# mauruszach/multimodal_diffusion

Hardware: AMD Instinct MI355X
Metric: denoising steps/sec @256x256 multimodal-cond batch=32 (higher is better)
Workload: dtype f32 via 3xbf16 split operands (6-term products, f32 accumulate; fp32-level error); 1 GPU; C3: 256x256 audio->video CFG denoising step (cond+null MMDiT d512 L8 H8 + noise head + DDIM), 384+37 tokens, batch 32 per GPU, DDIM 50 steps, guidance 3.5; global_batch=32, sampler_steps=50, parallelism=dp1, launch=eager, matmul=bf16x3, attn=default, cfg_halves=one stacked 2B batch, one stream

## Files before the change

multimodal_diffusion_amd/csrc/attn_bf16x3.hip:

```cpp
#include "avd_common.h"

#include <stdlib.h>
#include <type_traits>

namespace avd {

constexpr int A3_DH = 64, A3_KT = 64, A3_NW = 4;
constexpr float A3_NEG = -1.0e30f;

typedef short s16x4 __attribute__((ext_vector_type(4)));
typedef unsigned int u32x2 __attribute__((ext_vector_type(2)));
typedef float f32x4t __attribute__((ext_vector_type(4)));

#define AVD_LDS_PTR(p) ((__attribute__((address_space(3))) void*)(p))
#define AVD_GLB_PTR(p) ((const __attribute__((address_space(1))) void*)(p))

template <int TERMS> struct A3Terms;
template <> struct A3Terms<6> { static constexpr int N = 6; static constexpr int PA[6] = {2, 0, 1, 1, 0, 0}; static constexpr int PB[6] = {0, 2, 1, 0, 1, 0}; };
template <> struct A3Terms<9> { static constexpr int N = 9; static constexpr int PA[9] = {2, 2, 1, 2, 0, 1, 1, 0, 0}; static constexpr int PB[9] = {2, 1, 2, 0, 2, 1, 0, 1, 0}; };
template <> struct A3Terms<1> { static constexpr int N = 1; static constexpr int PA[1] = {0}; static constexpr int PB[1] = {0}; };
template <> struct A3Terms<3> { static constexpr int N = 3; static constexpr int PA[3] = {0, 1, 0}; static constexpr int PB[3] = {1, 0, 0}; };

template <bool SPLIT_OUT, int TERMS>
__global__ __launch_bounds__(A3_NW * 64, 2) void attn_bf16x3_kernel(const unsigned char* __restrict__ img, float* __restrict__ out,
                                                                    int Bt, int N, int Npad, int H, int n_query_max, int nqb,
                                                                    float s_inv2, float v_inv, float o_scale, RowSegs oseg) {
    constexpr int NW = A3_NW, ROWB = QKV3_ROWB;
    constexpr bool F16 = TERMS == 3;
    constexpr int NPL = s3_planes(TERMS);
    constexpr int PPW = 24 / NW;
    __shared__ __attribute__((aligned(16))) unsigned char Ks[A3_KT * ROWB];
    __shared__ __attribute__((aligned(16))) unsigned char Vs[A3_KT * ROWB];

    int qb, h, b;
    {
        const int nwg = gridDim.x, id = blockIdx.x, q = nwg >> 3, r = nwg & 7, x = id & 7;
        const int w = (x < r ? x * (q + 1) : r * (q + 1) + (x - r) * q) + (id >> 3);
        qb = w % nqb;
        h = (w / nqb) % H;
        b = w / (nqb * H);
    }
    const int seg_tok = oseg.tok[b < oseg.samples[0] ? 0 : 1], n_query = n_query_max < seg_tok ? n_query_max : seg_tok;
    if (qb * (A3_NW * 32) >= n_query) return;
    const int tid = threadIdx.x, lane = tid & 63, wave = tid >> 6;
    const int l31 = lane & 31, hi = lane >> 5;
    const int64_t hstride = (int64_t)Npad * ROWB;
    const unsigned char* Qb = img + (((int64_t)0 * Bt + b) * H + h) * hstride;
    const unsigned char* Kb = img + (((int64_t)1 * Bt + b) * H + h) * hstride;
    const unsigned char* Vb = img + (((int64_t)2 * Bt + b) * H + h) * hstride;

    const int q_row = qb * (NW * 32) + wave * 32 + l31;
    bf16x8 qf[4][3];
    {
        const unsigned char* src = Qb + (int64_t)(q_row < N ? q_row : N - 1) * ROWB + hi * 16;
#pragma unroll
        for (int s = 0; s < 4; ++s)
#pragma unroll
            for (int p = 0; p < NPL; ++p) qf[s][p] = *reinterpret_cast<const bf16x8*>(src + p * 128 + s * 32);
    }

    auto dma = [&](const unsigned char* gsrc, unsigned char* ldst, int kt) {
        const int last_row = N - 1 - kt * A3_KT;
#pragma unroll
        for (int i = 0; i < PPW; ++i) {
            const int p = wave + NW * i;
            const int off = p * 1024 + lane * 16;
            int row = off / ROWB;
            const int within = off - row * ROWB;
            row = row < last_row ? row : last_row;
            __builtin_amdgcn_global_load_lds(AVD_GLB_PTR(gsrc + ((int64_t)kt * A3_KT + row) * ROWB + within), AVD_LDS_PTR(ldst + p * 1024), 16,
                                             0, 0);
        }
    };

    f32x16 o0, o1;
#pragma unroll
    for (int r = 0; r < 16; ++r) { o0[r] = 0.f; o1[r] = 0.f; }
    float m_run = A3_NEG, l_run = 0.f;

    const int nkt = (N + A3_KT - 1) / A3_KT;
    dma(Kb, Ks, 0);
    dma(Vb, Vs, 0);
    __builtin_amdgcn_s_waitcnt(0x0f70);
    __syncthreads();

    const int ksw = (l31 >> 1) & 7;
    const int k_rd = l31 * ROWB;
    const int i16 = lane & 15, cb = (lane >> 4) & 1;
    const int v_q = i16 >> 2, v_p = i16 & 3;

    const bool active = qb * (NW * 32) + wave * 32 < n_query;
    for (int kt = 0; kt < nkt; ++kt) {
        const bool more = (kt + 1) < nkt;
        if (!active) {
            __builtin_amdgcn_s_waitcnt(0x0f70);
            __syncthreads();
            if (more) dma(Kb, Ks, kt + 1);
            __builtin_amdgcn_s_waitcnt(0x0f70);
            __syncthreads();
            if (more) dma(Vb, Vs, kt + 1);
            continue;
        }
        f32x16 s0, s1;
#pragma unroll
        for (int r = 0; r < 16; ++r) { s0[r] = 0.f; s1[r] = 0.f; }
        using TT = A3Terms<TERMS>;
#pragma unroll
        for (int s = 0; s < 4; ++s) {
            bf16x8 ka[3], kb2[3];
            const int ch = ((2 * s + hi) ^ ksw) << 4;
#pragma unroll
            for (int p = 0; p < NPL; ++p) {
                ka[p] = *reinterpret_cast<const bf16x8*>(Ks + k_rd + p * 128 + ch);
                kb2[p] = *reinterpret_cast<const bf16x8*>(Ks + k_rd + 32 * ROWB + p * 128 + ch);
            }
#pragma unroll
            for (int t = 0; t < TT::N; ++t) {
                s0 = mma16<F16>(ka[TT::PA[t]], qf[s][TT::PB[t]], s0);
                s1 = mma16<F16>(kb2[TT::PA[t]], qf[s][TT::PB[t]], s1);
            }
        }
        __builtin_amdgcn_s_waitcnt(0x0f70);
        __syncthreads();
        if (more) dma(Kb, Ks, kt + 1);

        if constexpr (F16) {
#pragma unroll
            for (int r = 0; r < 16; ++r) { s0[r] *= s_inv2; s1[r] *= s_inv2; }
        }
        if (!more && (N & (A3_KT - 1))) {
            const int kbase = kt * A3_KT;
#pragma unroll
            for (int r = 0; r < 16; ++r) {
                const int key = kbase + mfma32_row(r, hi);
                if (key >= N) s0[r] = A3_NEG;
                if (key + 32 >= N) s1[r] = A3_NEG;
            }
        }

        float mt = s0[0];
#pragma unroll
        for (int r = 1; r < 16; ++r) mt = fmaxf(mt, s0[r]);
#pragma unroll
        for (int r = 0; r < 16; ++r) mt = fmaxf(mt, s1[r]);
        mt = fmaxf(mt, __shfl_xor(mt, 32, 64));
        const float m_new = fmaxf(m_run, mt);
        const float m_sub = F16 ? m_new - 15.0f : m_new;
        float ps = 0.f;
#pragma unroll
        for (int r = 0; r < 16; ++r) {
            s0[r] = __builtin_amdgcn_exp2f(s0[r] - m_sub);
            s1[r] = __builtin_amdgcn_exp2f(s1[r] - m_sub);
            ps += s0[r] + s1[r];
        }
        if (__any(m_new > m_run)) {
            const float alpha = __builtin_amdgcn_exp2f(m_run - m_new);
// ... 272 lines not shown

    auto tile = [&](auto flags, int kt, f32x16& c0, f32x16& c1, f32x16& n0, f32x16& n1) {
        using FL = decltype(flags);
        constexpr bool MORE = FL::MORE;
        const float m_sub = F16 ? m_new - 15.0f : m_new;
        const float alpha = __builtin_amdgcn_exp2f(m_run - m_new);
        m_run = m_new;
        float ps = 0.f;
        constexpr int NSLOT_A = 4 * TT::N, NITEM_A = 28;
        auto item_a = [&](int w) {
            if (w < 16) {
                const float e0 = F16 ? c0[w] * s_inv2 : c0[w], e1 = F16 ? c1[w] * s_inv2 : c1[w];
                float p0 = __builtin_amdgcn_exp2f(e0 - m_sub), p1 = __builtin_amdgcn_exp2f(e1 - m_sub);
                ps += p0 + p1;
                asm volatile("" : "+v"(p0), "+v"(p1), "+v"(ps));
                c0[w] = p0;
                c1[w] = p1;
            } else if (w < 24) {
                const int r0 = (w - 16) * 2;
                float a0 = o0[r0] * alpha, a1 = o0[r0 + 1] * alpha, q0 = o1[r0] * alpha, q1 = o1[r0 + 1] * alpha;
                asm volatile("" : "+v"(a0), "+v"(a1), "+v"(q0), "+v"(q1));
                o0[r0] = a0; o0[r0 + 1] = a1;
                o1[r0] = q0; o1[r0 + 1] = q1;
            } else {
                split_pair(c0, c1, 0, w - 24, pf[0]);
                if constexpr (NPL == 3) asm volatile("" : "+v"(pf[0][0][w - 24]), "+v"(pf[0][1][w - 24]), "+v"(pf[0][2][w - 24]));
                else if constexpr (NPL == 2) asm volatile("" : "+v"(pf[0][0][w - 24]), "+v"(pf[0][1][w - 24]));
                else asm volatile("" : "+v"(pf[0][0][w - 24]));
            }
        };
        if constexpr (MORE) {
#pragma unroll
            for (int r = 0; r < 16; ++r) { n0[r] = 0.f; n1[r] = 0.f; }
#pragma unroll
            for (int sl = 0; sl < NSLOT_A; ++sl) {
                A3_SB();
                s_slot(n0, n1, sl / TT::N, sl % TT::N);
#pragma unroll
                for (int w = sl * NITEM_A / NSLOT_A; w < (sl + 1) * NITEM_A / NSLOT_A; ++w) item_a(w);
            }
            A3_SB();
            if constexpr (FL::VCL) {
                if (ragged) mask_tail(n0, n1, kt + 1);
            }
        } else {
#pragma unroll
            for (int w = 0; w < NITEM_A; ++w) item_a(w);
        }
        l_run = l_run * alpha + ps;
        sync();
        if constexpr (MORE) {
            if constexpr (FL::KCL) { if (kt + 2 < nkt) dma_clamp(Kb, Ks, kt + 2); }
            else if constexpr (!FL::VCL) dma_full(Kb, Ks, kt + 2);
        }

        float mt = A3_NEG;
#pragma unroll
        for (int g = 0; g < 4; ++g) {
#pragma unroll
            for (int sl = 0; sl < 2 * TT::N; ++sl) {
                A3_SB();
                pv_slot(g, sl / TT::N, sl % TT::N, pf[g & 1]);
                if (g < 3) {
                    constexpr int SPS = 2 * TT::N >= 4 ? 1 : 2;
#pragma unroll
                    for (int e = sl * SPS; e < (sl + 1) * SPS && e < 4; ++e) split_pair(c0, c1, g + 1, e, pf[(g + 1) & 1]);
                }
                if (MORE && g == 3) {
#pragma unroll
                    for (int w = sl * 16 / (2 * TT::N); w < (sl + 1) * 16 / (2 * TT::N); ++w) mt = fmaxf(mt, fmaxf(n0[w], n1[w]));
                    asm volatile("" : "+v"(mt));
                }
            }
        }
        A3_SB();
        if constexpr (MORE) {
            if constexpr (F16) mt *= s_inv2;
            mt = fmaxf(mt, __shfl_xor(mt, 32, 64));
            m_new = fmaxf(m_run, mt);
            if constexpr (FL::COPY) {
                c0 = n0;
                c1 = n1;
            }
            sync();
            if constexpr (FL::VCL) dma_clamp(Vb, Vs, kt + 1);
            else dma_full(Vb, Vs, kt + 1);
        }
    };
    {
        using Main = A3Flags<true, false, false, false>;
        using MainC = A3Flags<true, false, false, true>;
        using KClamp = A3Flags<true, true, false, true>;
        using VClamp = A3Flags<true, false, true, true>;
        using Last = A3Flags<false, false, false, false>;
        int kt = 0;
        for (; kt + 4 < nkt; kt += 2) {
            tile(Main{}, kt, sa0, sa1, sb0, sb1);
            tile(Main{}, kt + 1, sb0, sb1, sa0, sa1);
        }
        if (nkt - kt == 4) { tile(MainC{}, kt, sa0, sa1, sb0, sb1); ++kt; }
        if (nkt - kt == 3) { tile(KClamp{}, kt, sa0, sa1, sb0, sb1); ++kt; }
        if (nkt - kt == 2) { tile(VClamp{}, kt, sa0, sa1, sb0, sb1); ++kt; }
        tile(Last{}, kt, sa0, sa1, sb0, sb1);
    }
#undef A3_SB

    const float l_tot = l_run + __shfl_xor(l_run, 32, 64);
    const float inv = F16 ? v_inv / l_tot : 1.0f / l_tot;
    const int d = H * A3_DH;
    if constexpr (SPLIT_OUT) {
        float ch[8][4];
#pragma unroll
        for (int g4 = 0; g4 < 4; ++g4)
#pragma unroll
            for (int e = 0; e < 4; ++e) {
                ch[g4][e] = o0[4 * g4 + e] * inv;
                ch[4 + g4][e] = o1[4 * g4 + e] * inv;
            }
        unsigned char* o3 = reinterpret_cast<unsigned char*>(out);
#pragma unroll
        for (int c = 0; c < 8; c += 2) {
            float v[8];
#pragma unroll
            for (int e = 0; e < 4; ++e) {
                const float send = hi ? ch[c][e] : ch[c + 1][e];
                const float recv = __shfl_xor(send, 32, 64);
                v[e] = hi ? recv : ch[c][e];
                v[4 + e] = hi ? ch[c + 1][e] : recv;
            }
            if (q_row < n_query) {
                if constexpr (F16) store_split8_h2(o3, oseg.row(b, q_row), h * A3_DH + 8 * (c + hi), d, v, o_scale);
                else store_split8(o3, oseg.row(b, q_row), h * A3_DH + 8 * (c + hi), d, v);
            }
        }
    } else if (q_row < n_query) {
        float* dst = out + (oseg.row(b, q_row)) * d + h * A3_DH + 4 * hi;
#pragma unroll
        for (int g4 = 0; g4 < 4; ++g4) {
            f32x4 a = {o0[4 * g4] * inv, o0[4 * g4 + 1] * inv, o0[4 * g4 + 2] * inv, o0[4 * g4 + 3] * inv};
            f32x4 c = {o1[4 * g4] * inv, o1[4 * g4 + 1] * inv, o1[4 * g4 + 2] * inv, o1[4 * g4 + 3] * inv};
            *reinterpret_cast<f32x4*>(dst + 8 * g4) = a;
            *reinterpret_cast<f32x4*>(dst + 32 + 8 * g4) = c;
        }
    }
}

template <bool F16>
__device__ __forceinline__ f32x4t mma16s(bf16x8 a, bf16x8 b, f32x4t c) {
    if constexpr (F16) return __builtin_amdgcn_mfma_f32_16x16x32_f16(__builtin_bit_cast(f16x8, a), __builtin_bit_cast(f16x8, b), c, 0, 0, 0);
    else return __builtin_amdgcn_mfma_f32_16x16x32_bf16(a, b, c, 0, 0, 0);
}
int g_attn_m16 = 1;

struct S16 { f32x4t t[4][2]; };

template <bool SPLIT_OUT, int TERMS>
__global__ __launch_bounds__(A3_NW * 64, 2) void attn_bf16x3_p16_kernel(const unsigned char* __restrict__ img, float* __restrict__ out,
                                                                        int Bt, int N, int Npad, int H, int n_query_max, int nqb,
                                                                        float s_inv2, float v_inv, float o_scale, RowSegs oseg) {
    constexpr int NW = A3_NW, ROWB = QKV3_ROWB;
    constexpr bool F16 = TERMS == 3;
    constexpr int NPL = s3_planes(TERMS);
    constexpr int PPW = 24 / NW;
    using TT = A3Terms<TERMS>;
    __shared__ __attribute__((aligned(16))) unsigned char Ks[A3_KT * ROWB];
    __shared__ __attribute__((aligned(16))) unsigned char Vs[A3_KT * ROWB];

    int qb, h, b;
    {
        const int nwg = gridDim.x, id = blockIdx.x, q = nwg >> 3, r = nwg & 7, x = id & 7;
        const int w = (x < r ? x * (q + 1) : r * (q + 1) + (x - r) * q) + (id >> 3);
        qb = w % nqb;
        h = (w / nqb) % H;
        b = w / (nqb * H);
    }
    const int seg_tok = oseg.tok[b < oseg.samples[0] ? 0 : 1], n_query = n_query_max < seg_tok ? n_query_max : seg_tok;
    if (qb * (A3_NW * 32) >= n_query) return;
    const int tid = threadIdx.x, lane = tid & 63;
    const int wave = __builtin_amdgcn_readfirstlane(tid >> 6);
    const int l15 = lane & 15, kq = lane >> 4;
    const int64_t hstride = (int64_t)Npad * ROWB;
    const unsigned char* Qb = img + (((int64_t)0 * Bt + b) * H + h) * hstride;
    const unsigned char* Kb = img + (((int64_t)1 * Bt + b) * H + h) * hstride;
    const unsigned char* Vb = img + (((int64_t)2 * Bt + b) * H + h) * hstride;

    const int q_row0 = qb * (NW * 32) + wave * 32 + l15;
    bf16x8 qf[2][2][3];
#pragma unroll
    for (int qt = 0; qt < 2; ++qt) {
        const int qr = q_row0 + 16 * qt;
        const unsigned char* src = Qb + (int64_t)(qr < N ? qr : N - 1) * ROWB + kq * 16;
#pragma unroll
        for (int sd = 0; sd < 2; ++sd)
#pragma unroll
            for (int p = 0; p < NPL; ++p) qf[qt][sd][p] = *reinterpret_cast<const bf16x8*>(src + p * 128 + sd * 64);
    }
    auto dma_clamp = [&](const unsigned char* gsrc, unsigned char* ldst, int kt) {
        const int last_row = N - 1 - kt * A3_KT;
#pragma unroll
        for (int i = 0; i < PPW; ++i) {
            const int p = wave + NW * i;
            const int off = p * 1024 + lane * 16;
            int row = off / ROWB;
            const int within = off - row * ROWB;
            row = row < last_row ? row : last_row;
            __builtin_amdgcn_global_load_lds(AVD_GLB_PTR(gsrc + ((int64_t)kt * A3_KT + row) * ROWB + within), AVD_LDS_PTR(ldst + p * 1024), 16,
                                             0, 0);
        }
    };
    const unsigned lane16 = (unsigned)lane * 16u;
    auto dma_full = [&](const unsigned char* gsrc, unsigned char* ldst, int kt) {
        const unsigned char* base = gsrc + ((int64_t)kt * (A3_KT * ROWB) + wave * 1024);
#pragma unroll
        for (int i = 0; i < PPW; ++i)
            __builtin_amdgcn_global_load_lds(AVD_GLB_PTR(base + i * (NW * 1024) + lane16), AVD_LDS_PTR(ldst + (wave + NW * i) * 1024), 16, 0, 0);
    };
    auto sync = [&]() {
        __builtin_amdgcn_s_waitcnt(0x0f70);
        __syncthreads();
    };

    const int nkt = (N + A3_KT - 1) / A3_KT;
    const bool ragged = (N & (A3_KT - 1)) != 0;
    dma_clamp(Kb, Ks, 0);
    dma_clamp(Vb, Vs, 0);
    sync();

    const bool active = qb * (NW * 32) + wave * 32 < n_query;
    if (!active) {
        sync();
        if (nkt > 1) dma_clamp(Kb, Ks, 1);
        sync();
        for (int kt = 0; kt < nkt; ++kt) {
            sync();
            if (kt + 2 < nkt) dma_clamp(Kb, Ks, kt + 2);
            if (kt + 1 < nkt) {
                sync();
                dma_clamp(Vb, Vs, kt + 1);
            }
        }
        return;
    }

    const int ksw = (l15 >> 1) & 7;
    const int k_rd = l15 * ROWB;
    const int v_q = l15 >> 2, v_p = l15 & 3;
    const int v_key = 4 * kq + v_q;
    const int v_sw = qkv3_swizzle(2, v_key);
    const int v_rd = v_key * ROWB + 8 * (v_p & 1);
#define A3_SB() __builtin_amdgcn_sched_barrier(0)

    f32x4t o[4][2];
    S16 sa, sb;
#pragma unroll
    for (int i = 0; i < 4; ++i)
#pragma unroll
        for (int j = 0; j < 2; ++j) { o[i][j] = f32x4t{0.f, 0.f, 0.f, 0.f}; sa.t[i][j] = o[i][j]; sb.t[i][j] = o[i][j]; }
    float m_run[2] = {A3_NEG, A3_NEG}, l_run[2] = {0.f, 0.f}, m_new[2];

    bf16x8 ka[3];
    auto s_slot = [&](S16& d, int kt4, int sd, int t) {
        if (t == 0) {
            const int ch = ((4 * sd + kq) ^ ksw) << 4;
#pragma unroll
            for (int p = 0; p < NPL; ++p) ka[p] = *reinterpret_cast<const bf16x8*>(Ks + k_rd + kt4 * (16 * ROWB) + p * 128 + ch);
        }
        d.t[kt4][0] = mma16s<F16>(ka[TT::PA[t]], qf[0][sd][TT::PB[t]], d.t[kt4][0]);
        d.t[kt4][1] = mma16s<F16>(ka[TT::PA[t]], qf[1][sd][TT::PB[t]], d.t[kt4][1]);
    };
    auto mask_tail = [&](S16& d, int kt) {
        const int kbase = kt * A3_KT + 4 * kq;
#pragma unroll
        for (int i = 0; i < 4; ++i)
#pragma unroll
            for (int r = 0; r < 4; ++r)
                if (kbase + 16 * i + r >= N) { d.t[i][0][r] = A3_NEG; d.t[i][1][r] = A3_NEG; }
    };
    auto xmax = [&](float v) {
        const auto a = __builtin_amdgcn_permlane16_swap(__float_as_uint(v), __float_as_uint(v), false, false);
        v = fmaxf(__uint_as_float(a[0]), __uint_as_float(a[1]));
        const auto c = __builtin_amdgcn_permlane32_swap(__float_as_uint(v), __float_as_uint(v), false, false);
        return fmaxf(__uint_as_float(c[0]), __uint_as_float(c[1]));
    };
    auto xsum = [&](float v) {
        const auto a = __builtin_amdgcn_permlane16_swap(__float_as_uint(v), __float_as_uint(v), false, false);
        v = __uint_as_float(a[0]) + __uint_as_float(a[1]);
        const auto c = __builtin_amdgcn_permlane32_swap(__float_as_uint(v), __float_as_uint(v), false, false);
        return __uint_as_float(c[0]) + __uint_as_float(c[1]);
    };
    auto tile_max = [&](const S16& d, int qt) {
        float mt = A3_NEG;
#pragma unroll
        for (int i = 0; i < 4; ++i)
#pragma unroll
            for (int r = 0; r < 4; ++r) mt = fmaxf(mt, d.t[i][qt][r]);
        if constexpr (F16) mt *= s_inv2;
        return xmax(mt);
    };

#pragma unroll
    for (int i = 0; i < 4; ++i)
#pragma unroll
        for (int sd = 0; sd < 2; ++sd)
#pragma unroll
            for (int t = 0; t < TT::N; ++t) s_slot(sa, i, sd, t);
    if (nkt == 1 && ragged) mask_tail(sa, 0);
    sync();
    if (nkt > 1) dma_clamp(Kb, Ks, 1);
    m_new[0] = fmaxf(m_run[0], tile_max(sa, 0));
    m_new[1] = fmaxf(m_run[1], tile_max(sa, 1));
    sync();

    u32x4 pf[2][2][3];
    auto split_pair = [&](const S16& c, int g, int qt, int e, u32x4 (&dst)[3]) {
        const float a = c.t[2 * g + (e >> 1)][qt][2 * (e & 1)], cc = c.t[2 * g + (e >> 1)][qt][2 * (e & 1) + 1];
        if constexpr (F16) {
            const unsigned int hh = pk_f16(a, cc);
            const f32x2 u = unpk_f16(hh);
            dst[0][e] = hh;
            dst[1][e] = pk_f16(a - u[0], cc - u[1]);
        } else {
            const unsigned int hh = pk_bf16(a, cc);
            const float ra = a - bf16_lo(hh), rc = cc - bf16_hi(hh);
            dst[0][e] = hh;
            if constexpr (NPL > 1) {
                const unsigned int mm = pk_bf16(ra, rc);
                dst[1][e] = mm;
                dst[2][e] = pk_bf16(ra - bf16_lo(mm), rc - bf16_hi(mm));
            }
        }
    };
    bf16x8 vf[3];
    auto pv_slot = [&](int g, int dt, int tt, const u32x4 (&P)[2][3]) {
        if (tt == 0) {
            const int chunk = (2 * dt + (v_p >> 1)) ^ v_sw;
#pragma unroll
            for (int p = 0; p < NPL; ++p) {
                const unsigned char* a0 = Vs + v_rd + g * (32 * ROWB) + p * 128 + (chunk << 4);
                const s16x4 lo = __builtin_amdgcn_ds_read_tr16_b64_v4i16((__attribute__((address_space(3))) s16x4*)AVD_LDS_PTR(a0));
                const s16x4 up = __builtin_amdgcn_ds_read_tr16_b64_v4i16((__attribute__((address_space(3))) s16x4*)AVD_LDS_PTR(a0 + 16 * ROWB));
                const u32x2 a = __builtin_bit_cast(u32x2, lo), c2 = __builtin_bit_cast(u32x2, up);
                const u32x4 w = {a[0], a[1], c2[0], c2[1]};
                vf[p] = __builtin_bit_cast(bf16x8, w);
            }
        }
        o[dt][0] = mma16s<F16>(vf[TT::PA[tt]], __builtin_bit_cast(bf16x8, P[0][TT::PB[tt]]), o[dt][0]);
        o[dt][1] = mma16s<F16>(vf[TT::PA[tt]], __builtin_bit_cast(bf16x8, P[1][TT::PB[tt]]), o[dt][1]);
    };

    auto tile = [&](auto flags, int kt, S16& c, S16& n) {
        using FL = decltype(flags);
        constexpr bool MORE = FL::MORE;
        float m_sub[2], alpha[2], ps[2] = {0.f, 0.f};
#pragma unroll
        for (int qt = 0; qt < 2; ++qt) {
            m_sub[qt] = F16 ? m_new[qt] - 15.0f : m_new[qt];
            alpha[qt] = __builtin_amdgcn_exp2f(m_run[qt] - m_new[qt]);
            m_run[qt] = m_new[qt];
        }
        constexpr int NSLOT_A = 8 * TT::N, NITEM_A = 32;
        auto item_a = [&](int w) {
            if (w < 16) {
                const int i = w >> 2, qt = (w >> 1) & 1, r0 = 2 * (w & 1);
                const float e0 = F16 ? c.t[i][qt][r0] * s_inv2 : c.t[i][qt][r0], e1 = F16 ? c.t[i][qt][r0 + 1] * s_inv2 : c.t[i][qt][r0 + 1];
                float p0 = __builtin_amdgcn_exp2f(e0 - m_sub[qt]), p1 = __builtin_amdgcn_exp2f(e1 - m_sub[qt]);
                ps[qt] += p0 + p1;
                asm volatile("" : "+v"(p0), "+v"(p1), "+v"(ps[qt]));
                c.t[i][qt][r0] = p0;
                c.t[i][qt][r0 + 1] = p1;
            } else if (w < 24) {
                const int dt = (w - 16) >> 1, qt = (w - 16) & 1;
                float a0 = o[dt][qt][0] * alpha[qt], a1 = o[dt][qt][1] * alpha[qt], a2 = o[dt][qt][2] * alpha[qt], a3 = o[dt][qt][3] * alpha[qt];
                asm volatile("" : "+v"(a0), "+v"(a1), "+v"(a2), "+v"(a3));
                o[dt][qt] = f32x4t{a0, a1, a2, a3};
            } else {
                const int qt = (w - 24) >> 2, e = (w - 24) & 3;
                split_pair(c, 0, qt, e, pf[0][qt]);
                if constexpr (NPL == 3) asm volatile("" : "+v"(pf[0][qt][0][e]), "+v"(pf[0][qt][1][e]), "+v"(pf[0][qt][2][e]));
                else if constexpr (NPL == 2) asm volatile("" : "+v"(pf[0][qt][0][e]), "+v"(pf[0][qt][1][e]));
                else asm volatile("" : "+v"(pf[0][qt][0][e]));
            }
        };
        if constexpr (MORE) {
#pragma unroll
            for (int i = 0; i < 4; ++i)
#pragma unroll
                for (int j = 0; j < 2; ++j) n.t[i][j] = f32x4t{0.f, 0.f, 0.f, 0.f};
#pragma unroll
            for (int sl = 0; sl < NSLOT_A; ++sl) {
                A3_SB();
                s_slot(n, sl / (2 * TT::N), (sl / TT::N) & 1, sl % TT::N);
#pragma unroll
                for (int w = sl * NITEM_A / NSLOT_A; w < (sl + 1) * NITEM_A / NSLOT_A; ++w) item_a(w);
            }
            A3_SB();
            if constexpr (FL::VCL) {
                if (ragged) mask_tail(n, kt + 1);
            }
        } else {
#pragma unroll
            for (int w = 0; w < NITEM_A; ++w) item_a(w);
        }
        l_run[0] = l_run[0] * alpha[0] + ps[0];
        l_run[1] = l_run[1] * alpha[1] + ps[1];
        sync();
        if constexpr (MORE) {
            if constexpr (FL::KCL) { if (kt + 2 < nkt) dma_clamp(Kb, Ks, kt + 2); }
            else if constexpr (!FL::VCL) dma_full(Kb, Ks, kt + 2);
        }

        float mt[2] = {A3_NEG, A3_NEG};
#pragma unroll
        for (int g = 0; g < 2; ++g) {
#pragma unroll
            for (int sl = 0; sl < 4 * TT::N; ++sl) {
                A3_SB();
                pv_slot(g, sl / TT::N, sl % TT::N, pf[g]);
                if (g == 0) {
                    constexpr int NS = 4 * TT::N;
#pragma unroll
                    for (int w = sl * 8 / NS; w < (sl + 1) * 8 / NS; ++w) split_pair(c, 1, w >> 2, w & 3, pf[1][w >> 2]);
                }
                if (MORE && g == 1) {
                    constexpr int NS = 4 * TT::N;
#pragma unroll
                    for (int w = sl * 16 / NS; w < (sl + 1) * 16 / NS; ++w) {
                        const int i = w >> 2, qt = (w >> 1) & 1, r0 = 2 * (w & 1);
                        mt[qt] = fmaxf(mt[qt], fmaxf(n.t[i][qt][r0], n.t[i][qt][r0 + 1]));
                    }
                    asm volatile("" : "+v"(mt[0]), "+v"(mt[1]));
                }
            }
        }
        A3_SB();
        if constexpr (MORE) {
#pragma unroll
            for (int qt = 0; qt < 2; ++qt) {
                if constexpr (F16) mt[qt] *= s_inv2;
                m_new[qt] = fmaxf(m_run[qt], xmax(mt[qt]));
            }
            if constexpr (FL::COPY) c = n;
            sync();
            if constexpr (FL::VCL) dma_clamp(Vb, Vs, kt + 1);
            else dma_full(Vb, Vs, kt + 1);
        }
    };
    {
        using Main = A3Flags<true, false, false, false>;
        using MainC = A3Flags<true, false, false, true>;
        using KClamp = A3Flags<true, true, false, true>;
        using VClamp = A3Flags<true, false, true, true>;
        using Last = A3Flags<false, false, false, false>;
        int kt = 0;
        for (; kt + 4 < nkt; kt += 2) {
            tile(Main{}, kt, sa, sb);
            tile(Main{}, kt + 1, sb, sa);
        }
        if (nkt - kt == 4) { tile(MainC{}, kt, sa, sb); ++kt; }
        if (nkt - kt == 3) { tile(KClamp{}, kt, sa, sb); ++kt; }
        if (nkt - kt == 2) { tile(VClamp{}, kt, sa, sb); ++kt; }
        tile(Last{}, kt, sa, sb);
    }
#undef A3_SB

    float inv[2];
#pragma unroll
    for (int qt = 0; qt < 2; ++qt) {
        const float l_tot = xsum(l_run[qt]);
        inv[qt] = F16 ? v_inv / l_tot : 1.0f / l_tot;
    }
    const int d = H * A3_DH;
    const int q_row = q_row0 + 16 * (kq & 1);
    unsigned char* o3 = reinterpret_cast<unsigned char*>(out);
#pragma unroll
    for (int dt = 0; dt < 4; ++dt) {
        float v[8];
#pragma unroll
        for (int r = 0; r < 4; ++r) {
            const auto sw = __builtin_amdgcn_permlane16_swap(__float_as_uint(o[dt][0][r] * inv[0]), __float_as_uint(o[dt][1][r] * inv[1]), false, false);
            v[r] = __uint_as_float(sw[0]);
            v[4 + r] = __uint_as_float(sw[1]);
        }
        const int col = h * A3_DH + 16 * dt + 8 * (kq >> 1);
        if (q_row < n_query) {
            if constexpr (SPLIT_OUT) {
                if constexpr (F16) store_split8_h2(o3, oseg.row(b, q_row), col, d, v, o_scale);
                else store_split8(o3, oseg.row(b, q_row), col, d, v);
            } else {
                float* dst = out + (oseg.row(b, q_row)) * d + col;
                *reinterpret_cast<f32x4*>(dst) = f32x4{v[0], v[1], v[2], v[3]};
                *reinterpret_cast<f32x4*>(dst + 4) = f32x4{v[4], v[5], v[6], v[7]};
            }
        }
    }
}

int64_t qkv3_bytes(int B, int N, int H) { return (int64_t)3 * B * H * qkv3_npad(N) * QKV3_ROWB; }

template <int TERMS>
static void attn3_launch(const unsigned char* img, float* out, void* out3, int B, int N, int Npad, int H, int n_query, int nqb, hipStream_t st,
                         float img_scale, float out_scale, const RowSegs& oseg) {
    const float s_inv2 = 1.0f / (img_scale * img_scale), v_inv = 1.0f / img_scale;
    if (g_attn_m16 && (TERMS == 6 || TERMS == 9 || g_attn_m16 == 2)) {
        if (out3)
            hipLaunchKernelGGL((attn_bf16x3_p16_kernel<true, TERMS>), dim3(nqb * H * B), dim3(A3_NW * 64), 0, st, img, static_cast<float*>(out3),
                               B, N, Npad, H, n_query, nqb, s_inv2, v_inv, out_scale, oseg);
        else
            hipLaunchKernelGGL((attn_bf16x3_p16_kernel<false, TERMS>), dim3(nqb * H * B), dim3(A3_NW * 64), 0, st, img, out, B, N, Npad, H,
                               n_query, nqb, s_inv2, v_inv, out_scale, oseg);
        return;
    }
    if (g_attn_pipe == 2 || (g_attn_pipe == 1 && (TERMS == 6 || TERMS == 9))) {
        if (out3)
            hipLaunchKernelGGL((attn_bf16x3_pipe_kernel<true, TERMS>), dim3(nqb * H * B), dim3(A3_NW * 64), 0, st, img, static_cast<float*>(out3),
                               B, N, Npad, H, n_query, nqb, s_inv2, v_inv, out_scale, oseg);
        else
            hipLaunchKernelGGL((attn_bf16x3_pipe_kernel<false, TERMS>), dim3(nqb * H * B), dim3(A3_NW * 64), 0, st, img, out, B, N, Npad, H,
                               n_query, nqb, s_inv2, v_inv, out_scale, oseg);
        return;
    }
    if (out3)
        hipLaunchKernelGGL((attn_bf16x3_kernel<true, TERMS>), dim3(nqb * H * B), dim3(A3_NW * 64), 0, st, img, static_cast<float*>(out3), B, N,
                           Npad, H, n_query, nqb, s_inv2, v_inv, out_scale, oseg);
    else
        hipLaunchKernelGGL((attn_bf16x3_kernel<false, TERMS>), dim3(nqb * H * B), dim3(A3_NW * 64), 0, st, img, out, B, N, Npad, H, n_query, nqb,
                           s_inv2, v_inv, out_scale, oseg);
}

int attn_bf16x3(const void* qkv3, float* out, void* out3, int B, int N, int H, int n_query, int terms, hipStream_t st, float img_scale,
                float out_scale, int out_tokens, const RowSegs* out_rows) {
    const int out_tok = out_tokens > 0 ? out_tokens : N;
    AVD_REQUIRE(out_tok >= n_query, AVD_EINVAL, "attn_bf16x3: out_tokens=%d < n_query=%d", out_tok, n_query);
    AVD_REQUIRE(!out_rows || (out_rows->n_samples() == B && out_rows->samples[0] > 0 && out_rows->tok[0] > 0 && out_rows->tok[1] > 0 &&
                              out_rows->m0 == (int64_t)out_rows->samples[0] * out_rows->tok[0]), AVD_EINVAL,
                "attn_bf16x3: the output row layout does not hold the batch's %d samples", B);
    const RowSegs oseg = out_rows ? *out_rows : RowSegs::uniform(B, out_tok);
    AVD_REQUIRE(terms == 0 || terms == 6 || terms == 9 || terms == 1 || terms == 3, AVD_EINVAL, "attn_bf16x3: terms must be 6, 9, 1 or 3, got %d", terms);
    AVD_REQUIRE(img_scale > 0.f && img_scale < __builtin_inff() && out_scale > 0.f && out_scale < __builtin_inff() &&
                    img_scale * img_scale < __builtin_inff(), AVD_EINVAL, "attn_bf16x3: image scales must be positive and finite");
    AVD_REQUIRE(qkv3 && (out || out3), AVD_EINVAL, "attn_bf16x3: null pointer");
    AVD_REQUIRE(B > 0 && N > 0 && H > 0, AVD_EINVAL, "attn_bf16x3: bad dims B=%d N=%d H=%d", B, N, H);
    AVD_REQUIRE(n_query >= 0 && n_query <= N, AVD_EINVAL, "attn_bf16x3: n_query=%d outside [0,%d]", n_query, N);
    AVD_REQUIRE(aligned16(qkv3) && aligned16(out) && aligned16(out3), AVD_EUNSUPPORTED, "attn_bf16x3: pointers must be 16-byte aligned");
    AVD_REQUIRE(!out3 || (H * A3_DH) % 16 == 0, AVD_EUNSUPPORTED, "attn_bf16x3: split3 output needs d %% 16 == 0");
    if (n_query == 0) return AVD_OK;
    const int nqb = (n_query + 32 * A3_NW - 1) / (32 * A3_NW);
    AVD_REQUIRE((int64_t)B * H * nqb < (1ll << 31), AVD_EUNSUPPORTED, "attn_bf16x3: grid too large");
    const int tag = prof_tag_id("attn_bf16x3_kernel<%d>", terms ? terms : 6);
    ProfScope prof(tag, 4.0 * (double)B * H * (double)n_query * N * A3_DH, st);
    const int Npad = qkv3_npad(N);
    const auto* img = static_cast<const unsigned char*>(qkv3);
    if (terms == 9) attn3_launch<9>(img, out, out3, B, N, Npad, H, n_query, nqb, st, 1.f, 1.f, oseg);
    else if (terms == 1) attn3_launch<1>(img, out, out3, B, N, Npad, H, n_query, nqb, st, 1.f, 1.f, oseg);
    else if (terms == 3) attn3_launch<3>(img, out, out3, B, N, Npad, H, n_query, nqb, st, img_scale, out_scale, oseg);
    else attn3_launch<6>(img, out, out3, B, N, Npad, H, n_query, nqb, st, 1.f, 1.f, oseg);
    AVD_CHECK_LAUNCH("attn_bf16x3");
    return AVD_OK;
}

}

extern "C" int64_t avd_qkv3_bytes(int B, int N, int H) {
    if (B <= 0 || N <= 0 || H <= 0) return -1;
    return avd::qkv3_bytes(B, N, H);
}
extern "C" int avd_attn_fwd_qkv_f16x2_f32(const void* qkv, float* out, void* out2, int B, int N, int H, int n_query, float qkv_scale,
                                          float out_scale, avd_stream_t stream) {
    return avd::attn_bf16x3(qkv, out, out2, B, N, H, n_query, 3, static_cast<hipStream_t>(stream), qkv_scale, out_scale);
}
extern "C" int avd_attn_fwd_qkv3_f32(const void* qkv3, float* out, void* out3, int B, int N, int H, int n_query, int terms,
                                     avd_stream_t stream) {
    return avd::attn_bf16x3(qkv3, out, out3, B, N, H, n_query, terms, static_cast<hipStream_t>(stream));
}
```

Baseline: 121.0 steps/s.

## Specialize attention wave body for single query tile and skip ragged key pieces

Templates the per-wave attention body on the number of 16-row query tiles, so waves whose remaining queries fit in one tile skip the second tile's MFMAs, softmax and PV work. It also skips QK and PV sub-pieces whose keys lie entirely beyond the sequence in the final ragged tile. This targets wasted MFMA work on the ragged tail (421 tokens) at the cost of compiling two kernel bodies, which raises code size and instruction-cache pressure.

```diff
diff --git a/multimodal_diffusion_amd/csrc/attn_bf16x3.hip b/multimodal_diffusion_amd/csrc/attn_bf16x3.hip
--- a/multimodal_diffusion_amd/csrc/attn_bf16x3.hip
+++ b/multimodal_diffusion_amd/csrc/attn_bf16x3.hip
@@ -2,6 +2,7 @@
 
 #include <stdlib.h>
 #include <type_traits>
+#include <utility>
 
 namespace avd {
 
@@ -580,7 +581,12 @@
 }
 int g_attn_m16 = 1;
 
-struct S16 { f32x4t t[4][2]; };
+template <int NQT> struct S16 { f32x4t t[4][NQT]; };
+template <int V> using IC = std::integral_constant<int, V>;
+template <class F, int... I>
+__device__ __forceinline__ void a3_unrolled_seq(F&& f, std::integer_sequence<int, I...>) { (f(IC<I>{}), ...); }
+template <int N, class F>
+__device__ __forceinline__ void a3_unrolled(F&& f) { a3_unrolled_seq(f, std::make_integer_sequence<int, N>{}); }
 
 template <bool SPLIT_OUT, int TERMS>
 __global__ __launch_bounds__(A3_NW * 64, 2) void attn_bf16x3_p16_kernel(const unsigned char* __restrict__ img, float* __restrict__ out,
@@ -613,9 +619,11 @@
     const unsigned char* Vb = img + (((int64_t)2 * Bt + b) * H + h) * hstride;
 
     const int q_row0 = qb * (NW * 32) + wave * 32 + l15;
+    const bool one_qt = n_query - (qb * (NW * 32) + wave * 32) <= 16;
     bf16x8 qf[2][2][3];
 #pragma unroll
     for (int qt = 0; qt < 2; ++qt) {
+        if (qt == 1 && one_qt) break;
         const int qr = q_row0 + 16 * qt;
         const unsigned char* src = Qb + (int64_t)(qr < N ? qr : N - 1) * ROWB + kq * 16;
 #pragma unroll
@@ -677,250 +685,327 @@
     const int v_sw = qkv3_swizzle(2, v_key);
     const int v_rd = v_key * ROWB + 8 * (v_p & 1);
 #define A3_SB() __builtin_amdgcn_sched_barrier(0)
-
-    f32x4t o[4][2];
-    S16 sa, sb;
-#pragma unroll
-    for (int i = 0; i < 4; ++i)
-#pragma unroll
-        for (int j = 0; j < 2; ++j) { o[i][j] = f32x4t{0.f, 0.f, 0.f, 0.f}; sa.t[i][j] = o[i][j]; sb.t[i][j] = o[i][j]; }
-    float m_run[2] = {A3_NEG, A3_NEG}, l_run[2] = {0.f, 0.f}, m_new[2];
-
-    bf16x8 ka[3];
-    auto s_slot = [&](S16& d, int kt4, int sd, int t) {
-        if (t == 0) {
-            const int ch = ((4 * sd + kq) ^ ksw) << 4;
-#pragma unroll
-            for (int p = 0; p < NPL; ++p) ka[p] = *reinterpret_cast<const bf16x8*>(Ks + k_rd + kt4 * (16 * ROWB) + p * 128 + ch);
-        }
-        d.t[kt4][0] = mma16s<F16>(ka[TT::PA[t]], qf[0][sd][TT::PB[t]], d.t[kt4][0]);
-        d.t[kt4][1] = mma16s<F16>(ka[TT::PA[t]], qf[1][sd][TT::PB[t]], d.t[kt4][1]);
-    };
-    auto mask_tail = [&](S16& d, int kt) {
-        const int kbase = kt * A3_KT + 4 * kq;
+    const int v_last = N - (nkt - 1) * A3_KT;
+
+    auto wave_body = [&](auto nqt_c) __attribute__((always_inline)) {
+        constexpr int NQT = decltype(nqt_c)::value;
+        asm volatile("; query tiles %0" ::"n"(NQT));
+        using S16T = S16<NQT>;
+        f32x4t o[4][NQT];
+        S16T sa, sb;
 #pragma unroll
         for (int i = 0; i < 4; ++i)
 #pragma unroll
-            for (int r = 0; r < 4; ++r)
-                if (kbase + 16 * i + r >= N) { d.t[i][0][r] = A3_NEG; d.t[i][1][r] = A3_NEG; }
-    };
-    auto xmax = [&](float v) {
-        const auto a = __builtin_amdgcn_permlane16_swap(__float_as_uint(v), __float_as_uint(v), false, false);
-        v = fmaxf(__uint_as_float(a[0]), __uint_as_float(a[1]));
-        const auto c = __builtin_amdgcn_permlane32_swap(__float_as_uint(v), __float_as_uint(v), false, false);
-        return fmaxf(__uint_as_float(c[0]), __uint_as_float(c[1]));
-    };
-    auto xsum = [&](float v) {
-        const auto a = __builtin_amdgcn_permlane16_swap(__float_as_uint(v), __float_as_uint(v), false, false);
-        v = __uint_as_float(a[0]) + __uint_as_float(a[1]);
-        const auto c = __builtin_amdgcn_permlane32_swap(__float_as_uint(v), __float_as_uint(v), false, false);
-        return __uint_as_float(c[0]) + __uint_as_float(c[1]);
-    };
-    auto tile_max = [&](const S16& d, int qt) {
-        float mt = A3_NEG;
-#pragma unroll
-        for (int i = 0; i < 4; ++i)
-#pragma unroll
-            for (int r = 0; r < 4; ++r) mt = fmaxf(mt, d.t[i][qt][r]);
-        if constexpr (F16) mt *= s_inv2;
-        return xmax(mt);
-    };
-
-#pragma unroll
-    for (int i = 0; i < 4; ++i)
-#pragma unroll
-        for (int sd = 0; sd < 2; ++sd)
-#pragma unroll
-            for (int t = 0; t < TT::N; ++t) s_slot(sa, i, sd, t);
-    if (nkt == 1 && ragged) mask_tail(sa, 0);
-    sync();
-    if (nkt > 1) dma_clamp(Kb, Ks, 1);
-    m_new[0] = fmaxf(m_run[0], tile_max(sa, 0));
-    m_new[1] = fmaxf(m_run[1], tile_max(sa, 1));
-    sync();
-
-    u32x4 pf[2][2][3];
-    auto split_pair = [&](const S16& c, int g, int qt, int e, u32x4 (&dst)[3]) {
-        const float a = c.t[2 * g + (e >> 1)][qt][2 * (e & 1)], cc = c.t[2 * g + (e >> 1)][qt][2 * (e & 1) + 1];
-        if constexpr (F16) {
-            const unsigned int hh = pk_f16(a, cc);
-            const f32x2 u = unpk_f16(hh);
-            dst[0][e] = hh;
-            dst[1][e] = pk_f16(a - u[0], cc - u[1]);
+            for (int j = 0; j < NQT; ++j) { o[i][j] = f32x4t{0.f, 0.f, 0.f, 0.f}; sa.t[i][j] = o[i][j]; sb.t[i][j] = o[i][j]; }
+        float m_run[NQT], l_run[NQT], m_new[NQT];
+#pragma unroll
+        for (int qt = 0; qt < NQT; ++qt) { m_run[qt] = A3_NEG; l_run[qt] = 0.f; }
+
+        bf16x8 ka[3];
+        auto s_slot = [&](S16T& d, int kt4, int sd, int t) {
+            if (t == 0) {
+                const int ch = ((4 * sd + kq) ^ ksw) << 4;
+#pragma unroll
+                for (int p = 0; p < NPL; ++p) ka[p] = *reinterpret_cast<const bf16x8*>(Ks + k_rd + kt4 * (16 * ROWB) + p * 128 + ch);
+            }
+            d.t[kt4][0] = mma16s<F16>(ka[TT::PA[t]], qf[0][sd][TT::PB[t]], d.t[kt4][0]);
+            if constexpr (NQT == 2) d.t[kt4][1] = mma16s<F16>(ka[TT::PA[t]], qf[1][sd][TT::PB[t]], d.t[kt4][1]);
+        };
+        auto mask_tail = [&](S16T& d, int kt) {
+            const int kbase = kt * A3_KT + 4 * kq;
+#pragma unroll
+            for (int i = 0; i < 4; ++i)
+#pragma unroll
+                for (int r = 0; r < 4; ++r)
+                    if (kbase + 16 * i + r >= N) {
+#pragma unroll
+                        for (int qt = 0; qt < NQT; ++qt) d.t[i][qt][r] = A3_NEG;
+                    }
+        };
+        auto xmax = [&](float v) {
+            const auto a = __builtin_amdgcn_permlane16_swap(__float_as_uint(v), __float_as_uint(v), false, false);
+            v = fmaxf(__uint_as_float(a[0]), __uint_as_float(a[1]));
+            const auto c = __builtin_amdgcn_permlane32_swap(__float_as_uint(v), __float_as_uint(v), false, false);
+            return fmaxf(__uint_as_float(c[0]), __uint_as_float(c[1]));
+        };
+        auto xsum = [&](float v) {
+            const auto a = __builtin_amdgcn_permlane16_swap(__float_as_uint(v), __float_as_uint(v), false, false);
+            v = __uint_as_float(a[0]) + __uint_as_float(a[1]);
+            const auto c = __builtin_amdgcn_permlane32_swap(__float_as_uint(v), __float_as_uint(v), false, false);
+            return __uint_as_float(c[0]) + __uint_as_float(c[1]);
+        };
+        auto tile_max = [&](const S16T& d, int qt) {
+            float mt = A3_NEG;
+#pragma unroll
+            for (int i = 0; i < 4; ++i)
+#pragma unroll
+                for (int r = 0; r < 4; ++r) mt = fmaxf(mt, d.t[i][qt][r]);
+            if constexpr (F16) mt *= s_inv2;
+            return xmax(mt);
+        };
+
+        auto s_piece = [&](S16T& d, int i) __attribute__((always_inline)) {
+#pragma unroll
+            for (int sd = 0; sd < 2; ++sd)
+#pragma unroll
+                for (int t = 0; t < TT::N; ++t) s_slot(d, i, sd, t);
+        };
+        if (nkt > 1 || v_last > 3 * 16) {
+#pragma unroll
+            for (int i = 0; i < 4; ++i) s_piece(sa, i);
         } else {
-            const unsigned int hh = pk_bf16(a, cc);
-            const float ra = a - bf16_lo(hh), rc = cc - bf16_hi(hh);
-            dst[0][e] = hh;
-            if constexpr (NPL > 1) {
-                const unsigned int mm = pk_bf16(ra, rc);
-                dst[1][e] = mm;
-                dst[2][e] = pk_bf16(ra - bf16_lo(mm), rc - bf16_hi(mm));
-            }
-        }
-    };
-    bf16x8 vf[3];
-    auto pv_slot = [&](int g, int dt, int tt, const u32x4 (&P)[2][3]) {
-        if (tt == 0) {
-            const int chunk = (2 * dt + (v_p >> 1)) ^ v_sw;
-#pragma unroll
-            for (int p = 0; p < NPL; ++p) {
-                const unsigned char* a0 = Vs + v_rd + g * (32 * ROWB) + p * 128 + (chunk << 4);
-                const s16x4 lo = __builtin_amdgcn_ds_read_tr16_b64_v4i16((__attribute__((address_space(3))) s16x4*)AVD_LDS_PTR(a0));
-                const s16x4 up = __builtin_amdgcn_ds_read_tr16_b64_v4i16((__attribute__((address_space(3))) s16x4*)AVD_LDS_PTR(a0 + 16 * ROWB));
-                const u32x2 a = __builtin_bit_cast(u32x2, lo), c2 = __builtin_bit_cast(u32x2, up);
-                const u32x4 w = {a[0], a[1], c2[0], c2[1]};
-                vf[p] = __builtin_bit_cast(bf16x8, w);
-            }
-        }
-        o[dt][0] = mma16s<F16>(vf[TT::PA[tt]], __builtin_bit_cast(bf16x8, P[0][TT::PB[tt]]), o[dt][0]);
-        o[dt][1] = mma16s<F16>(vf[TT::PA[tt]], __builtin_bit_cast(bf16x8, P[1][TT::PB[tt]]), o[dt][1]);
-    };
-
-    auto tile = [&](auto flags, int kt, S16& c, S16& n) {
-        using FL = decltype(flags);
-        constexpr bool MORE = FL::MORE;
-        float m_sub[2], alpha[2], ps[2] = {0.f, 0.f};
-#pragma unroll
-        for (int qt = 0; qt < 2; ++qt) {
-            m_sub[qt] = F16 ? m_new[qt] - 15.0f : m_new[qt];
-            alpha[qt] = __builtin_amdgcn_exp2f(m_run[qt] - m_new[qt]);
-            m_run[qt] = m_new[qt];
-        }
-        constexpr int NSLOT_A = 8 * TT::N, NITEM_A = 32;
-        auto item_a = [&](int w) {
-            if (w < 16) {
-                const int i = w >> 2, qt = (w >> 1) & 1, r0 = 2 * (w & 1);
-                const float e0 = F16 ? c.t[i][qt][r0] * s_inv2 : c.t[i][qt][r0], e1 = F16 ? c.t[i][qt][r0 + 1] * s_inv2 : c.t[i][qt][r0 + 1];
-                float p0 = __builtin_amdgcn_exp2f(e0 - m_sub[qt]), p1 = __builtin_amdgcn_exp2f(e1 - m_sub[qt]);
-                ps[qt] += p0 + p1;
-                asm volatile("" : "+v"(p0), "+v"(p1), "+v"(ps[qt]));
-                c.t[i][qt][r0] = p0;
-                c.t[i][qt][r0 + 1] = p1;
-            } else if (w < 24) {
-                const int dt = (w - 16) >> 1, qt = (w - 16) & 1;
-                float a0 = o[dt][qt][0] * alpha[qt], a1 = o[dt][qt][1] * alpha[qt], a2 = o[dt][qt][2] * alpha[qt], a3 = o[dt][qt][3] * alpha[qt];
-                asm volatile("" : "+v"(a0), "+v"(a1), "+v"(a2), "+v"(a3));
-                o[dt][qt] = f32x4t{a0, a1, a2, a3};
+            s_piece(sa, 0);
+#pragma unroll
+            for (int i = 1; i < 3; ++i)
+                if (16 * i < v_last) s_piece(sa, i);
+        }
+        if (nkt == 1 && ragged) mask_tail(sa, 0);
+        sync();
+        if (nkt > 1) dma_clamp(Kb, Ks, 1);
+#pragma unroll
+        for (int qt = 0; qt < NQT; ++qt) m_new[qt] = fmaxf(m_run[qt], tile_max(sa, qt));
+        sync();
+
+        u32x4 pf[2][NQT][3];
+        auto split_pair = [&](const S16T& c, int g, int qt, int e, u32x4 (&dst)[3]) {
+            const float a = c.t[2 * g + (e >> 1)][qt][2 * (e & 1)], cc = c.t[2 * g + (e >> 1)][qt][2 * (e & 1) + 1];
+            if constexpr (F16) {
+                const unsigned int hh = pk_f16(a, cc);
+                const f32x2 u = unpk_f16(hh);
+                dst[0][e] = hh;
+                dst[1][e] = pk_f16(a - u[0], cc - u[1]);
             } else {
-                const int qt = (w - 24) >> 2, e = (w - 24) & 3;
-                split_pair(c, 0, qt, e, pf[0][qt]);
-                if constexpr (NPL == 3) asm volatile("" : "+v"(pf[0][qt][0][e]), "+v"(pf[0][qt][1][e]), "+v"(pf[0][qt][2][e]));
-                else if constexpr (NPL == 2) asm volatile("" : "+v"(pf[0][qt][0][e]), "+v"(pf[0][qt][1][e]));
-                else asm volatile("" : "+v"(pf[0][qt][0][e]));
+                const unsigned int hh = pk_bf16(a, cc);
+                const float ra = a - bf16_lo(hh), rc = cc - bf16_hi(hh);
+                dst[0][e] = hh;
+                if constexpr (NPL > 1) {
+                    const unsigned int mm = pk_bf16(ra, rc);
+                    dst[1][e] = mm;
+                    dst[2][e] = pk_bf16(ra - bf16_lo(mm), rc - bf16_hi(mm));
+                }
             }
         };
-        if constexpr (MORE) {
-#pragma unroll
-            for (int i = 0; i < 4; ++i)
-#pragma unroll
-                for (int j = 0; j < 2; ++j) n.t[i][j] = f32x4t{0.f, 0.f, 0.f, 0.f};
-#pragma unroll
-            for (int sl = 0; sl < NSLOT_A; ++sl) {
+        auto zero_pairs = [&](int g, int e0) __attribute__((always_inline)) {
+#pragma unroll
+            for (int qt = 0; qt < NQT; ++qt)
+#pragma unroll
+                for (int p = 0; p < NPL; ++p) { pf[g][qt][p][e0] = 0u; pf[g][qt][p][e0 + 1] = 0u; }
+        };
+        bf16x8 vf[3];
+        auto pv_slot = [&](int g, int dt, int tt, const u32x4 (&P)[NQT][3]) {
+            if (tt == 0) {
+                const int chunk = (2 * dt + (v_p >> 1)) ^ v_sw;
+#pragma unroll
+                for (int p = 0; p < NPL; ++p) {
+                    const unsigned char* a0 = Vs + v_rd + g * (32 * ROWB) + p * 128 + (chunk << 4);
+                    const s16x4 lo = __builtin_amdgcn_ds_read_tr16_b64_v4i16((__attribute__((address_space(3))) s16x4*)AVD_LDS_PTR(a0));
+                    const s16x4 up = __builtin_amdgcn_ds_read_tr16_b64_v4i16((__attribute__((address_space(3))) s16x4*)AVD_LDS_PTR(a0 + 16 * ROWB));
+                    const u32x2 a = __builtin_bit_cast(u32x2, lo), c2 = __builtin_bit_cast(u32x2, up);
+                    const u32x4 w = {a[0], a[1], c2[0], c2[1]};
+                    vf[p] = __builtin_bit_cast(bf16x8, w);
+                }
+            }
+            o[dt][0] = mma16s<F16>(vf[TT::PA[tt]], __builtin_bit_cast(bf16x8, P[0][TT::PB[tt]]), o[dt][0]);
+            if constexpr (NQT == 2) o[dt][1] = mma16s<F16>(vf[TT::PA[tt]], __builtin_bit_cast(bf16x8, P[1][TT::PB[tt]]), o[dt][1]);
+        };
+
+        auto tile = [&](auto flags, int kt, S16T& c, S16T& n) __attribute__((always_inline)) {
+            using FL = decltype(flags);
+            constexpr bool MORE = FL::MORE;
+            float m_sub[NQT], alpha[NQT], ps[NQT];
+#pragma unroll
+            for (int qt = 0; qt < NQT; ++qt) {
+                ps[qt] = 0.f;
+                m_sub[qt] = F16 ? m_new[qt] - 15.0f : m_new[qt];
+                alpha[qt] = __builtin_amdgcn_exp2f(m_run[qt] - m_new[qt]);
+                m_run[qt] = m_new[qt];
+            }
+            constexpr int NSLOT_A = 8 * TT::N, NITEM_A = 32;
+            auto item_a = [&](int w) {
+                if (w < 16) {
+                    const int i = w >> 2, qt = (w >> 1) & 1, r0 = 2 * (w & 1);
+                    if (qt >= NQT) return;
+                    const float e0 = F16 ? c.t[i][qt][r0] * s_inv2 : c.t[i][qt][r0], e1 = F16 ? c.t[i][qt][r0 + 1] * s_inv2 : c.t[i][qt][r0 + 1];
+                    float p0 = __builtin_amdgcn_exp2f(e0 - m_sub[qt]), p1 = __builtin_amdgcn_exp2f(e1 - m_sub[qt]);
+                    ps[qt] += p0 + p1;
+                    asm volatile("" : "+v"(p0), "+v"(p1), "+v"(ps[qt]));
+                    c.t[i][qt][r0] = p0;
+                    c.t[i][qt][r0 + 1] = p1;
+                } else if (w < 24) {
+                    const int dt = (w - 16) >> 1, qt = (w - 16) & 1;
+                    if (qt >= NQT) return;
+                    float a0 = o[dt][qt][0] * alpha[qt], a1 = o[dt][qt][1] * alpha[qt], a2 = o[dt][qt][2] * alpha[qt], a3 = o[dt][qt][3] * alpha[qt];
+                    asm volatile("" : "+v"(a0), "+v"(a1), "+v"(a2), "+v"(a3));
+                    o[dt][qt] = f32x4t{a0, a1, a2, a3};
+                } else {
+                    const int qt = (w - 24) >> 2, e = (w - 24) & 3;
+                    if (qt >= NQT) return;
+                    split_pair(c, 0, qt, e, pf[0][qt]);
+                    if constexpr (NPL == 3) asm volatile("" : "+v"(pf[0][qt][0][e]), "+v"(pf[0][qt][1][e]), "+v"(pf[0][qt][2][e]));
+                    else if constexpr (NPL == 2) asm volatile("" : "+v"(pf[0][qt][0][e]), "+v"(pf[0][qt][1][e]));
+                    else asm volatile("" : "+v"(pf[0][qt][0][e]));
+                }
+            };
+            if constexpr (MORE) {
+#pragma unroll
+                for (int i = 0; i < 4; ++i)
+#pragma unroll
+                    for (int j = 0; j < NQT; ++j) n.t[i][j] = f32x4t{0.f, 0.f, 0.f, 0.f};
+                auto piece_slots = [&](auto i, auto mfma) __attribute__((always_inline)) {
+                    constexpr int PS = 2 * TT::N;
+                    a3_unrolled<PS>([&](auto s) __attribute__((always_inline)) {
+                        constexpr int sl = i * PS + s;
+                        if constexpr (decltype(mfma)::value) {
+                            A3_SB();
+                            s_slot(n, sl / (2 * TT::N), (sl / TT::N) & 1, sl % TT::N);
+                        }
+#pragma unroll
+                        for (int w = sl * NITEM_A / NSLOT_A; w < (sl + 1) * NITEM_A / NSLOT_A; ++w) item_a(w);
+                    });
+                };
+                auto piece = [&](auto i) __attribute__((always_inline)) {
+                    if constexpr (FL::VCL && i > 0) {
+                        if (16 * i < v_last) piece_slots(i, std::true_type{});
+                        else piece_slots(i, std::false_type{});
+                    } else {
+                        piece_slots(i, std::true_type{});
+                    }
+                };
+                piece(IC<0>{});
+                piece(IC<1>{});
+                piece(IC<2>{});
+                piece(IC<3>{});
                 A3_SB();
-                s_slot(n, sl / (2 * TT::N), (sl / TT::N) & 1, sl % TT::N);
-#pragma unroll
-                for (int w = sl * NITEM_A / NSLOT_A; w < (sl + 1) * NITEM_A / NSLOT_A; ++w) item_a(w);
-            }
+                if constexpr (FL::VCL) {
+                    if (ragged) mask_tail(n, kt + 1);
+                }
+            } else {
+#pragma unroll
+                for (int i = 0; i < 4; ++i)
+                    if (i == 0 || 16 * i < v_last) {
+#pragma unroll
+                        for (int w = 4 * i; w < 4 * i + 4; ++w) item_a(w);
+                    }
+#pragma unroll
+                for (int w = 16; w < 24; ++w) item_a(w);
+#pragma unroll
+                for (int g = 0; g < 2; ++g) {
+#pragma unroll
+                    for (int half = 0; half < 2; ++half) {
+                        if (g == 1 && v_last <= 32) {
+                        } else if ((g == 0 && half == 0) || 16 * (2 * g + half) < v_last) {
+#pragma unroll
+                            for (int qt = 0; qt < NQT; ++qt)
+#pragma unroll
+                                for (int e = 2 * half; e < 2 * half + 2; ++e) split_pair(c, g, qt, e, pf[g][qt]);
+                        } else {
+                            zero_pairs(g, 2 * half);
+                        }
+                    }
+                }
+            }
+#pragma unroll
+            for (int qt = 0; qt < NQT; ++qt) l_run[qt] = l_run[qt] * alpha[qt] + ps[qt];
+            sync();
+            if constexpr (MORE) {
+                if constexpr (FL::KCL) { if (kt + 2 < nkt) dma_clamp(Kb, Ks, kt + 2); }
+                else if constexpr (!FL::VCL) dma_full(Kb, Ks, kt + 2);
+            }
+
+            float mt[NQT];
+#pragma unroll
+            for (int qt = 0; qt < NQT; ++qt) mt[qt] = A3_NEG;
+            auto pv_group = [&](auto g) __attribute__((always_inline)) {
+                a3_unrolled<4 * TT::N>([&](auto s) __attribute__((always_inline)) {
+                    constexpr int sl = s;
+                    A3_SB();
+                    pv_slot(g, sl / TT::N, sl % TT::N, pf[g]);
+                    if (MORE && g == 0) {
+                        constexpr int NS = 4 * TT::N;
+#pragma unroll
+                        for (int w = sl * 8 / NS; w < (sl + 1) * 8 / NS; ++w)
+                            if ((w >> 2) < NQT) split_pair(c, 1, w >> 2, w & 3, pf[1][w >> 2]);
+                    }
+                    if (MORE && g == 1) {
+                        constexpr int NS = 4 * TT::N;
+#pragma unroll
+                        for (int w = sl * 16 / NS; w < (sl + 1) * 16 / NS; ++w) {
+                            const int i = w >> 2, qt = (w >> 1) & 1, r0 = 2 * (w & 1);
+                            if (qt < NQT) mt[qt] = fmaxf(mt[qt], fmaxf(n.t[i][qt][r0], n.t[i][qt][r0 + 1]));
+                        }
+                        if constexpr (NQT == 2) asm volatile("" : "+v"(mt[0]), "+v"(mt[1]));
+                        else asm volatile("" : "+v"(mt[0]));
+                    }
+                });
+            };
+            pv_group(IC<0>{});
+            if (MORE || 32 < v_last) pv_group(IC<1>{});
             A3_SB();
-            if constexpr (FL::VCL) {
-                if (ragged) mask_tail(n, kt + 1);
-            }
-        } else {
-#pragma unroll
-            for (int w = 0; w < NITEM_A; ++w) item_a(w);
-        }
-        l_run[0] = l_run[0] * alpha[0] + ps[0];
-        l_run[1] = l_run[1] * alpha[1] + ps[1];
-        sync();
-        if constexpr (MORE) {
-            if constexpr (FL::KCL) { if (kt + 2 < nkt) dma_clamp(Kb, Ks, kt + 2); }
-            else if constexpr (!FL::VCL) dma_full(Kb, Ks, kt + 2);
-        }
-
-        float mt[2] = {A3_NEG, A3_NEG};
-#pragma unroll
-        for (int g = 0; g < 2; ++g) {
-#pragma unroll
-            for (int sl = 0; sl < 4 * TT::N; ++sl) {
-                A3_SB();
-                pv_slot(g, sl / TT::N, sl % TT::N, pf[g]);
-                if (g == 0) {
-                    constexpr int NS = 4 * TT::N;
-#pragma unroll
-                    for (int w = sl * 8 / NS; w < (sl + 1) * 8 / NS; ++w) split_pair(c, 1, w >> 2, w & 3, pf[1][w >> 2]);
+            if constexpr (MORE) {
+#pragma unroll
+                for (int qt = 0; qt < NQT; ++qt) {
+                    if constexpr (F16) mt[qt] *= s_inv2;
+                    m_new[qt] = fmaxf(m_run[qt], xmax(mt[qt]));
                 }
-                if (MORE && g == 1) {
-                    constexpr int NS = 4 * TT::N;
-#pragma unroll
-                    for (int w = sl * 16 / NS; w < (sl + 1) * 16 / NS; ++w) {
-                        const int i = w >> 2, qt = (w >> 1) & 1, r0 = 2 * (w & 1);
-                        mt[qt] = fmaxf(mt[qt], fmaxf(n.t[i][qt][r0], n.t[i][qt][r0 + 1]));
-                    }
-                    asm volatile("" : "+v"(mt[0]), "+v"(mt[1]));
+                if constexpr (FL::COPY) c = n;
+                sync();
+                if constexpr (FL::VCL) dma_clamp(Vb, Vs, kt + 1);
+                else dma_full(Vb, Vs, kt + 1);
+            }
+        };
+        {
+            using Main = A3Flags<true, false, false, false>;
+            using MainC = A3Flags<true, false, false, true>;
+            using KClamp = A3Flags<true, true, false, true>;
+            using VClamp = A3Flags<true, false, true, true>;
+            using Last = A3Flags<false, false, false, false>;
+            int kt = 0;
+            for (; kt + 4 < nkt; kt += 2) {
+                tile(Main{}, kt, sa, sb);
+                tile(Main{}, kt + 1, sb, sa);
+            }
+            if (nkt - kt == 4) { tile(MainC{}, kt, sa, sb); ++kt; }
+            if (nkt - kt == 3) { tile(KClamp{}, kt, sa, sb); ++kt; }
+            if (nkt - kt == 2) { tile(VClamp{}, kt, sa, sb); ++kt; }
+            tile(Last{}, kt, sa, sb);
+        }
+
+        float inv[NQT];
+#pragma unroll
+        for (int qt = 0; qt < NQT; ++qt) {
+            const float l_tot = xsum(l_run[qt]);
+            inv[qt] = F16 ? v_inv / l_tot : 1.0f / l_tot;
+        }
+        const int d = H * A3_DH;
+        const int q_row = q_row0 + 16 * (kq & 1);
+        unsigned char* o3 = reinterpret_cast<unsigned char*>(out);
+#pragma unroll
+        for (int dt = 0; dt < 4; ++dt) {
+            float v[8];
+#pragma unroll
+            for (int r = 0; r < 4; ++r) {
+                float t1 = 0.f;
+                if constexpr (NQT == 2) t1 = o[dt][1][r] * inv[1];
+                const auto sw = __builtin_amdgcn_permlane16_swap(__float_as_uint(o[dt][0][r] * inv[0]), __float_as_uint(t1), false, false);
+                v[r] = __uint_as_float(sw[0]);
+                v[4 + r] = __uint_as_float(sw[1]);
+            }
+            const int col = h * A3_DH + 16 * dt + 8 * (kq >> 1);
+            if (q_row < n_query) {
+                if constexpr (SPLIT_OUT) {
+                    if constexpr (F16) store_split8_h2(o3, oseg.row(b, q_row), col, d, v, o_scale);
+                    else store_split8(o3, oseg.row(b, q_row), col, d, v);
+                } else {
+                    float* dst = out + (oseg.row(b, q_row)) * d + col;
+                    *reinterpret_cast<f32x4*>(dst) = f32x4{v[0], v[1], v[2], v[3]};
+                    *reinterpret_cast<f32x4*>(dst + 4) = f32x4{v[4], v[5], v[6], v[7]};
                 }
             }
         }
-        A3_SB();
-        if constexpr (MORE) {
-#pragma unroll
-            for (int qt = 0; qt < 2; ++qt) {
-                if constexpr (F16) mt[qt] *= s_inv2;
-                m_new[qt] = fmaxf(m_run[qt], xmax(mt[qt]));
-            }
-            if constexpr (FL::COPY) c = n;
-            sync();
-            if constexpr (FL::VCL) dma_clamp(Vb, Vs, kt + 1);
-            else dma_full(Vb, Vs, kt + 1);
-        }
-    };
-    {
-        using Main = A3Flags<true, false, false, false>;
-        using MainC = A3Flags<true, false, false, true>;
-        using KClamp = A3Flags<true, true, false, true>;
-        using VClamp = A3Flags<true, false, true, true>;
-        using Last = A3Flags<false, false, false, false>;
-        int kt = 0;
-        for (; kt + 4 < nkt; kt += 2) {
-            tile(Main{}, kt, sa, sb);
-            tile(Main{}, kt + 1, sb, sa);
-        }
-        if (nkt - kt == 4) { tile(MainC{}, kt, sa, sb); ++kt; }
-        if (nkt - kt == 3) { tile(KClamp{}, kt, sa, sb); ++kt; }
-        if (nkt - kt == 2) { tile(VClamp{}, kt, sa, sb); ++kt; }
-        tile(Last{}, kt, sa, sb);
-    }
+    };
 #undef A3_SB
-
-    float inv[2];
-#pragma unroll
-    for (int qt = 0; qt < 2; ++qt) {
-        const float l_tot = xsum(l_run[qt]);
-        inv[qt] = F16 ? v_inv / l_tot : 1.0f / l_tot;
-    }
-    const int d = H * A3_DH;
-    const int q_row = q_row0 + 16 * (kq & 1);
-    unsigned char* o3 = reinterpret_cast<unsigned char*>(out);
-#pragma unroll
-    for (int dt = 0; dt < 4; ++dt) {
-        float v[8];
-#pragma unroll
-        for (int r = 0; r < 4; ++r) {
-            const auto sw = __builtin_amdgcn_permlane16_swap(__float_as_uint(o[dt][0][r] * inv[0]), __float_as_uint(o[dt][1][r] * inv[1]), false, false);
-            v[r] = __uint_as_float(sw[0]);
-            v[4 + r] = __uint_as_float(sw[1]);
-        }
-        const int col = h * A3_DH + 16 * dt + 8 * (kq >> 1);
-        if (q_row < n_query) {
-            if constexpr (SPLIT_OUT) {
-                if constexpr (F16) store_split8_h2(o3, oseg.row(b, q_row), col, d, v, o_scale);
-                else store_split8(o3, oseg.row(b, q_row), col, d, v);
-            } else {
-                float* dst = out + (oseg.row(b, q_row)) * d + col;
-                *reinterpret_cast<f32x4*>(dst) = f32x4{v[0], v[1], v[2], v[3]};
-                *reinterpret_cast<f32x4*>(dst + 4) = f32x4{v[4], v[5], v[6], v[7]};
-            }
-        }
-    }
+    if (one_qt) wave_body(IC<1>{});
+    else wave_body(IC<2>{});
 }
 
 int64_t qkv3_bytes(int B, int N, int H) { return (int64_t)3 * B * H * qkv3_npad(N) * QKV3_ROWB; }
```

Result: no change. 121.2 steps/s (median of 6 runs) (+0.2%).
